# raguilar011095/planet_heightmap_generation

Measured on AMD Instinct MI355X. Metric: Mcells·iter/s, terrain-post erosion stack, higher is better.
Workload: dtype f64

## Files before the change

planet_heightmap_generation_amd/csrc/flood_host.cc:

```cpp
#include <algorithm>
#include <atomic>
#include <chrono>
#include <cmath>
#include <cstdint>
#include <cstdio>
#include <cstdlib>
#include <cstring>
#include <string>
#include <thread>
#include <stdexcept>
#include <vector>

#include "host_util.h"
#include "wo_internal.h"

namespace wo {

namespace {

inline double cell_noise(int32_t r) { return flood_cell_noise_of(r); }

using HeapItem = FloodHeapItem;
struct KeyHeap {
    hvec<HeapItem>& d;
// ... 270 lines not shown
}
void build_land_index(int32_t N, const uint8_t* ocean, FloodScratch& S) {
    S.landIndex.resize(N);
    parallel_ranges(N, [&](int64_t b, int64_t e, int) { for (int64_t r = b; r < e; ++r) S.landIndex[r] = -1; });
    parallel_ranges(S.L, [&](int64_t b, int64_t e, int) { for (int64_t i = b; i < e; ++i) S.landIndex[S.landCell[i]] = (int32_t)i; });
    filter_ranges(N, S.landByR, [&](int64_t r) { return !ocean[r]; }, [&](int64_t r) { return S.landIndex[r]; });
}
void build_compact_csr(const int32_t* off, const int32_t* adj, const uint8_t* ocean, FloodScratch& S) {
    const int32_t L = S.L;
    S.offL.assign(L + 1, 0);
    parallel_ranges(L, [&](int64_t b, int64_t e, int) {
        for (int64_t i = b; i < e; ++i) {
            const int32_t r = S.landCell[i];
            int32_t c = 0;
            for (int32_t j = off[r]; j < off[r + 1]; ++j) if (!ocean[adj[j]]) ++c;
            S.offL[i + 1] = c;
        }
    });
    inclusive_scan_parallel(S.offL.data() + 1, L);
    S.adjL.resize(S.offL[L]);
    parallel_ranges(L, [&](int64_t b, int64_t e, int) {
        for (int64_t i = b; i < e; ++i) {
            const int32_t r = S.landCell[i];
            int32_t o = S.offL[i];
            for (int32_t j = off[r]; j < off[r + 1]; ++j) { const int32_t nb = adj[j]; if (!ocean[nb]) S.adjL[o++] = S.landIndex[nb]; }
        }
    });
}
void find_seeds(int32_t N, const int32_t* off, const int32_t* adj, const uint8_t* ocean, const int32_t* label, int32_t mainLab, FloodScratch& S) {
    S.seedCell.clear();
    std::vector<std::vector<int32_t>> part(host_threads() + 1);
    parallel_ranges(N, [&](int64_t b, int64_t e, int t) {
        for (int64_t r = b; r < e; ++r) {
            if (ocean[r]) continue;
            for (int32_t j = off[r]; j < off[r + 1]; ++j) {
                const int32_t nb = adj[j];
                if (ocean[nb] && label[nb] == mainLab) { part[t].push_back(S.landIndex[r]); break; }
            }
        }
    });
    for (auto& v : part) S.seedCell.insert(S.seedCell.end(), v.begin(), v.end());
}
void build_landmass_cells(const int32_t* comp, const int32_t* compIndex, FloodScratch& S) {
    const int32_t nComp = (int32_t)S.compSize.size();
    S.compCellStart.assign(nComp + 1, 0);
    for (int32_t k = 0; k < nComp; ++k) S.compCellStart[k + 1] = S.compCellStart[k] + S.compSize[k];
    S.compCells.resize(S.compCellStart[nComp]);
    const int nt = host_threads() + 2;
    std::vector<int32_t> cnt((size_t)nt * (size_t)std::max(nComp, 1), 0);
    int usedRanges = 0;
    parallel_ranges(S.L, [&](int64_t b, int64_t e, int t) {
        int32_t* c = cnt.data() + (size_t)t * (size_t)nComp;
        for (int64_t q = b; q < e; ++q) { const int32_t k = compIndex[comp[S.landByR[q]]]; if (k >= 0) ++c[k]; }
        int cur = usedRanges; while (cur < t + 1 && !__atomic_compare_exchange_n(&usedRanges, &cur, t + 1, false, __ATOMIC_RELAXED, __ATOMIC_RELAXED)) {}
    });
    for (int32_t k = 0; k < nComp; ++k) {
        int32_t at = S.compCellStart[k];
        for (int t = 0; t < usedRanges; ++t) { int32_t& c = cnt[(size_t)t * (size_t)nComp + k]; const int32_t n = c; c = at; at += n; }
    }
    parallel_ranges(S.L, [&](int64_t b, int64_t e, int t) {
        int32_t* c = cnt.data() + (size_t)t * (size_t)nComp;
        for (int64_t q = b; q < e; ++q) { const int32_t i = S.landByR[q]; const int32_t k = compIndex[comp[i]]; if (k >= 0) S.compCells[c[k]++] = i; }
    });
}
void build_landmasses(FloodScratch& S) {
    const int32_t L = S.L;
    hvec<int32_t> comp((size_t)L);
    mesh_components(L, S.offL.data(), S.adjL.data(), [](int32_t) { return true; }, [](int32_t, int32_t) { return true; }, comp.data());
    hvec<int32_t> size((size_t)L);
    parallel_ranges(L, [&](int64_t b, int64_t e, int) { std::memset(size.data() + b, 0, sizeof(int32_t) * (size_t)(e - b)); });
    parallel_ranges(L, [&](int64_t b, int64_t e, int) { for_runs(b, e, comp.data(), [](int64_t) { return true; }, [&](int32_t root, int64_t cnt) { __atomic_fetch_add(&size[root], (int32_t)cnt, __ATOMIC_RELAXED); }); });
    const int32_t nS = (int32_t)S.seedCell.size();
    std::vector<int32_t> ord(nS);
    for (int32_t k = 0; k < nS; ++k) ord[k] = k;
    std::stable_sort(ord.begin(), ord.end(), [&](int32_t a, int32_t b) {
        const int32_t ca = comp[S.seedCell[a]], cb = comp[S.seedCell[b]];
        return size[ca] != size[cb] ? size[ca] > size[cb] : ca < cb;
    });
    S.compSeeds.assign(ord.begin(), ord.end());
    S.compSeedStart.clear(); S.compSize.clear();
    for (int32_t k = 0; k < nS; ++k)
        if (k == 0 || comp[S.seedCell[ord[k]]] != comp[S.seedCell[ord[k - 1]]]) { S.compSeedStart.push_back(k); S.compSize.push_back(size[comp[S.seedCell[ord[k]]]]); }
    S.compSeedStart.push_back(nS);
    S.stamp.resize(L);
    const int32_t nComp = (int32_t)S.compSize.size();
    hvec<int32_t>& compIndex = size;
    parallel_ranges(L, [&](int64_t b, int64_t e, int) { for (int64_t i = b; i < e; ++i) compIndex[i] = -1; });
    S.seedLocal.assign(nS, 0);
    for (int32_t k = 0; k < nComp; ++k) {
        compIndex[comp[S.seedCell[ord[S.compSeedStart[k]]]]] = k;
        for (int32_t q = S.compSeedStart[k]; q < S.compSeedStart[k + 1]; ++q) S.seedLocal[ord[q]] = q - S.compSeedStart[k];
    }
    build_landmass_cells(comp.data(), compIndex.data(), S);
}
}

void flood_build_static(int32_t N, const int32_t* off, const int32_t* adj, const float* xyz, const uint8_t* ocean, FloodScratch& S, const int32_t* mortonAll) {
    FloodTimer T(std::getenv("WO_FLOOD_TIMING") != nullptr, "[flood static]", 12);
    hvec<int32_t> label((size_t)N);
    const int32_t mainLab = main_ocean_label(N, off, adj, ocean, label.data());
    T.lap("ocean labels");
    build_land_list(N, xyz, ocean, mortonAll, S.landCell);
    T.lap("morton sort");
    const int32_t L = S.L = (int32_t)S.landCell.size();
    build_land_index(N, ocean, S);
    build_compact_csr(off, adj, ocean, S);
    T.lap("compact csr");
// ... 245 lines not shown
    j.aboveGroup = j.kx > ct.level;
    j.sameSurface = std::memcmp(&j.altSurface, &x.surface, 4) == 0;
    j.ordered = x.drain >= 0 && st[x.drain].surface < x.surface && st[ct.other].surface < x.surface;
    return j;
}
bool flood_pass1_landmasses(FloodScratch& S, FloodTieReport& rep) {
    FloodTimer T(S);
    const int32_t nComp = (int32_t)S.compSize.size();
    const int nt = flood_workers(nComp);
    rep = FloodTieReport{};
    rep.landmasses = nComp; rep.workers = nt;
    if (nComp == 0) return true;
    parallel_ranges(S.L, [&](int64_t b, int64_t en, int) { std::memset(S.stamp.data() + b, 0, sizeof(int32_t) * (size_t)(en - b)); });
    if ((int)S.workerHeaps.size() < nt) S.workerHeaps.resize(nt);
    std::vector<std::vector<Contest>> contests(nt);
    std::vector<int64_t> ng(nt, 0), nn(nt, 0);
    std::atomic<int32_t> next{0};
    auto worker = [&](int w) {
        for (;;) {
            const int32_t k = next.fetch_add(1);
            if (k >= nComp) break;
            walk_landmass(S, seeded_walk(S, k, S.workerHeaps[w], contests[w], ng[w], nn[w]));
        }
    };
    run_on_threads(nt, worker);
    for (int w = 0; w < nt; ++w) {
        rep.groups += ng[w]; rep.nested += nn[w];
        for (const Contest& ct : contests[w]) {
            ++rep.contested;
            if (ct.other >= 0 && judge_contest(S, ct).open()) { ++rep.openParents; rep.alt.push_back({ct.cell, ct.other}); }
            else ++rep.unresolved;
        }
    }
    T.lap("pass1 par");
    if (T.on) std::fprintf(stderr, "[flood] landmasses %d, workers %d, tie groups %lld (nested %lld), contested %lld, open parents %lld, unresolved %lld\n",
                           rep.landmasses, rep.workers, (long long)rep.groups, (long long)rep.nested, (long long)rep.contested, (long long)rep.openParents, (long long)rep.unresolved);
    return rep.unresolved == 0;
}
}

void flood_import_pass1(const int32_t* par, const float* surface, const int32_t* root, FloodScratch& S) {
    FloodCell* st = S.state.data();
    parallel_ranges(S.L, [&](int64_t b, int64_t en, int) {
        for (int64_t i = b; i < en; ++i) {
            const int32_t p = par[i];
            st[i].drain = (p == -2) ? TO_OCEAN : (p == -1 ? UNVISITED : p);
            st[i].surface = surface[i];
            st[i].root = (p == -1) ? -1 : root[i];
        }
    });
}

namespace {
struct TreeCtx { const FloodCell* st; float* eL; const float* surface; double carveStrength; uint8_t* onPath; int32_t* localIdx = nullptr; int32_t chainsMin = 0; };

struct ChainScratch {
    std::vector<int32_t> par, kids, kidStart, order, sz, heavy, posOf, headPos, jump, cellAt, depth;
    std::vector<float> E, S;
    std::vector<double> term;
};
bool tree_pass2_chains(const TreeCtx& X, const int32_t* cells, int32_t n, int64_t& lenSum, int64_t& nDeficit) {
    const double EPS = 1e-7;
    static thread_local ChainScratch C;
    const FloodCell* st = X.st;
    float* eL = X.eL;
    int32_t* loc = X.localIdx;
    const double carveStrength = X.carveStrength;
    auto surf = [&](int32_t i) { return X.surface ? X.surface[i] : st[i].surface; };
    for (int32_t q = 0; q < n; ++q) loc[cells[q]] = q;
    C.par.resize(n); C.kidStart.assign((size_t)n + 1, 0);
    int32_t rootQ = -1, nRoots = 0;
    for (int32_t q = 0; q < n; ++q) {
        const int32_t d = st[cells[q]].drain;
        if (d >= 0) { const int32_t pq = loc[d]; if (pq < 0 || pq >= n || cells[pq] != d) return false; C.par[q] = pq; ++C.kidStart[pq + 1]; }
        else { C.par[q] = -1; rootQ = q; ++nRoots; }
    }
    if (nRoots != 1) return false;
    if (surf(cells[rootQ]) < 0) return false;
    for (int32_t q = 0; q < n; ++q) C.kidStart[q + 1] += C.kidStart[q];
    C.kids.resize(n); C.order.resize(n);
    {
        std::vector<int32_t>& fill = C.sz; fill.assign(C.kidStart.begin(), C.kidStart.end() - 1);
        for (int32_t q = 0; q < n; ++q) if (C.par[q] >= 0) C.kids[fill[C.par[q]]++] = q;
        int32_t head = 0, tail = 0;
        C.order[tail++] = rootQ;
        while (head < tail) { const int32_t v = C.order[head++]; for (int32_t j = C.kidStart[v]; j < C.kidStart[v + 1]; ++j) C.order[tail++] = C.kids[j]; }
        if (tail != n) return false;
    }
    C.sz.assign(n, 1); C.heavy.assign(n, -1);
    for (int32_t i = n - 1; i > 0; --i) { const int32_t v = C.order[i]; C.sz[C.par[v]] += C.sz[v]; }
    for (int32_t i = 1; i < n; ++i) { const int32_t v = C.order[i], p = C.par[v]; if (C.heavy[p] < 0 || C.sz[v] > C.sz[C.heavy[p]]) C.heavy[p] = v; }
    C.posOf.resize(n); C.headPos.resize(n); C.jump.assign(n, -1); C.cellAt.resize(n); C.E.resize(n); C.S.resize(n); C.depth.resize(n);
    C.depth[rootQ] = 0;
    for (int32_t i = 1; i < n; ++i) { const int32_t v = C.order[i]; C.depth[v] = C.depth[C.par[v]] + 1; }
    {
        int32_t base = 0;
        for (int32_t i = 0; i < n; ++i) {
            const int32_t v = C.order[i];
            if (C.par[v] >= 0 && C.heavy[C.par[v]] == v) continue;
            int32_t m = 0;
            for (int32_t u = v; u >= 0; u = C.heavy[u]) ++m;
            const int32_t top = base + m - 1;
            int32_t at = top;
            for (int32_t u = v; u >= 0; u = C.heavy[u], --at) { C.posOf[u] = at; C.headPos[at] = top; C.cellAt[at] = cells[u]; C.E[at] = eL[cells[u]]; C.S[at] = surf(cells[u]); }
            C.jump[top] = C.par[v] >= 0 ? C.posOf[C.par[v]] : -1;
            base += m;
        }
// ... 23 lines not shown
                    if (!whole && S[p] <= peakElev) { scanning = false; break; }
                    if (E[p] > peakElev) { peakElev = E[p]; peakIdx = seen + (p - a); }
                }
                if (!scanning) {
                    const double rcs = std::ceil((double)len * 0.3);
                    const int32_t rad = rcs > 3.0 ? (int32_t)rcs : 3;
                    need = peakIdx + rad + 1 < len ? peakIdx + rad + 1 : len;
                }
            }
            seen += b - a + 1;
            a = jump[b];
        }
        if (X.onPath) for (int s = 0; s < nseg; ++s) for (int32_t p = segA[s]; p <= segB[s]; ++p) X.onPath[C.cellAt[p]] = 1;
        lenSum += len;
        if (peakIdx < 0) continue;
        const double carveAmount = deficit * carveStrength;
        const double rc = std::ceil((double)len * 0.3);
        const int32_t radius = rc > 3.0 ? (int32_t)rc : 3;
        const int32_t k0 = peakIdx - radius > 0 ? peakIdx - radius : 0;
        const int32_t k1 = peakIdx + radius < len - 1 ? peakIdx + radius : len - 1;
        const int32_t m = k1 - k0 + 1;
        if ((int32_t)C.term.size() < m) C.term.resize((size_t)m + 256);
        double* term = C.term.data();
        for (int32_t i = 0; i < m; ++i) term[i] = 1 - std::fabs((double)(k0 + i - peakIdx)) / (radius + 1);
        double kernelSum = 0;
        for (int32_t i = 0; i < m; ++i) kernelSum += term[i];
        if (kernelSum > 0) {
            for (int s = 0; s < nseg; ++s) {
                const int32_t ks = segK[s], ke = ks + (segB[s] - segA[s]);
                const int32_t lo = k0 > ks ? k0 : ks, hi = k1 < ke ? k1 : ke;
                float* Es = E + (segA[s] - ks);
                const double* ts = term - k0;
                for (int32_t k = lo; k <= hi; ++k) {
                    const double w = ts[k] / kernelSum;
                    float v = (float)((double)Es[k] - carveAmount * w);
                    if (v < 0) v = 0;
                    Es[k] = v;
                }
            }
        }
        E[pr] = (float)((double)E[pr] + deficit * (1 - carveStrength));
    }
    for (int32_t q = 0; q < n; ++q) eL[cells[q]] = E[C.posOf[q]];
    return true;
}

void tree_pass23(const TreeCtx& X, int32_t* cells, int32_t n, std::vector<int32_t>& path, int64_t& lenSum, int64_t& nDeficit) {
    const double EPS = 1e-7;
    const FloodCell* st = X.st;
    float* eL = X.eL;
    const double carveStrength = X.carveStrength;
    uint8_t* onPath = X.onPath;
    auto surf = [&](int32_t i) { return X.surface ? X.surface[i] : st[i].surface; };
    const bool chained = X.localIdx && X.chainsMin > 0 && n >= X.chainsMin && tree_pass2_chains(X, cells, n, lenSum, nDeficit);

    for (int32_t q = 0; q < n && !chained; ++q) {
        const int32_t r = cells[q];
        const double deficit = (double)surf(r) - (double)eL[r];
        if (deficit <= EPS) continue;
        ++nDeficit;
        path.clear();
        int32_t peakIdx = -1;
        double peakElev = -INFINITY;
        for (int32_t cur = r; cur >= 0; cur = st[cur].drain) {
            path.push_back(cur);
            if ((double)eL[cur] > peakElev) { peakElev = eL[cur]; peakIdx = (int32_t)path.size() - 1; }
        }
        if (onPath) for (int32_t c : path) onPath[c] = 1;
        const int32_t len = (int32_t)path.size();
        lenSum += len;
        if (peakIdx < 0) continue;
        const double carveAmount = deficit * carveStrength;
        const double rc = std::ceil((double)len * 0.3);
        const int32_t radius = rc > 3.0 ? (int32_t)rc : 3;
        const int32_t k0 = peakIdx - radius > 0 ? peakIdx - radius : 0;
        const int32_t k1 = peakIdx + radius < len - 1 ? peakIdx + radius : len - 1;
        double kernelSum = 0;
        for (int32_t k = k0; k <= k1; ++k) kernelSum += 1 - std::fabs((double)(k - peakIdx)) / (radius + 1);
        if (kernelSum > 0) {
            for (int32_t k = k0; k <= k1; ++k) {
                const double w = (1 - std::fabs((double)(k - peakIdx)) / (radius + 1)) / kernelSum;
                float v = (float)((double)eL[path[k]] - carveAmount * w);
                if (v < 0) v = 0;
                eL[path[k]] = v;
            }
        }
        eL[r] = (float)((double)eL[r] + deficit * (1 - carveStrength));
    }
    if (n > 1) {
        if (n <= 2048) {
            std::stable_sort(cells, cells + n, [&](int32_t a, int32_t b) { return asc_bits(surf(a)) < asc_bits(surf(b)); });
        } else {
            std::vector<uint32_t> k0(n), k1(n); std::vector<int32_t> c1(n);
            for (int32_t i = 0; i < n; ++i) k0[i] = asc_bits(surf(cells[i]));
            uint32_t* ka = k0.data(); uint32_t* kb = k1.data(); int32_t* ca = cells; int32_t* cb = c1.data();
            for (int pass = 0; pass < 3; ++pass) {
                const int sh = pass * 11; const uint32_t mask = pass == 2 ? 1023u : 2047u;
                uint32_t cnt[2049]; std::memset(cnt, 0, sizeof(cnt));
                for (int32_t i = 0; i < n; ++i) cnt[((ka[i] >> sh) & mask) + 1]++;
                for (int i = 0; i < 2048; ++i) cnt[i + 1] += cnt[i];
                for (int32_t i = 0; i < n; ++i) { const uint32_t d = cnt[(ka[i] >> sh) & mask]++; kb[d] = ka[i]; cb[d] = ca[i]; }
                std::swap(ka, kb); std::swap(ca, cb);
            }
            if (ca != cells) std::memcpy(cells, ca, sizeof(int32_t) * (size_t)n);
        }
    }
    for (int32_t q = 0; q < n; ++q) {
        const int32_t c = cells[q], t = st[c].drain;
        if (t == NO_TARGET || t == UNVISITED) continue;
        const double te = (t == TO_OCEAN) ? 0.0 : (double)eL[t];
        if ((double)eL[c] <= te) eL[c] = (float)(te + EPS);
    }
}
void cut_chunks(const std::vector<int32_t>& cnt, int32_t nTrees, int64_t budget, std::vector<int32_t>& chunkStart) {
    chunkStart.assign(1, 0);
    for (int32_t t = 0, last = 0; t < nTrees; ++t)
        if (cnt[t + 1] - cnt[last] >= budget) { chunkStart.push_back(t + 1); last = t + 1; }
    if (chunkStart.back() != nTrees) chunkStart.push_back(nTrees);
}
bool open_parent_is_harmless(const FloodScratch& S, int32_t x, int32_t p1) {
    const FloodCell* st = S.state.data(); const float* eL = S.eL.data();
    const int32_t p0 = st[x].drain;
    const bool untouched = !S.onPath[x] && std::memcmp(&eL[x], &st[x].e, 4) == 0;
    const double h = (double)st[x].e;
    return untouched && p0 >= 0 && h > (double)eL[p0] && h > (double)eL[p1];
}
void write_back(float* e, const FloodScratch& S) {
    const int32_t* landCell = S.landCell.data(); const float* eL = S.eL.data();
    if (S.landOrder) parallel_ranges(S.L, [&](int64_t b, int64_t en, int) { std::memcpy(e + b, eL + b, sizeof(float) * (size_t)(en - b)); });
    else parallel_ranges(S.L, [&](int64_t b, int64_t en, int) { for (int64_t i = b; i < en; ++i) e[landCell[i]] = eL[i]; });
}
void group_land_by_tree(FloodScratch& S, std::vector<int32_t>& cnt2) {
    const int32_t L = S.L, nTrees = (int32_t)S.seedCell.size();
    const int32_t* root = S.root.data(); const int32_t* byR = S.landByR.data(); int32_t* list2 = S.list2.data();
    cnt2.assign(nTrees + 1, 0);
    const int T = (int)std::max<int64_t>(1, std::min<int64_t>({(int64_t)host_threads(), 16, (int64_t)L / 65536 + 1}));
    std::vector<int32_t> cw((size_t)nTrees * T, 0);
    auto share = [&](int t, int64_t& b, int64_t& e) { b = (int64_t)L * t / T; e = (int64_t)L * (t + 1) / T; };
    std::vector<std::thread> th;
    for (int t = 0; t < T; ++t) th.emplace_back([&, t]() {
        int64_t b, e; share(t, b, e);
        for (int64_t k = b; k < e; ++k) { const int32_t r = root[byR[k]]; if (r >= 0) ++cw[(size_t)r * T + t]; }
    });
    for (auto& x : th) x.join();
    int32_t run = 0;
    for (int32_t tr = 0; tr < nTrees; ++tr) {
        cnt2[tr] = run;
        for (int t = 0; t < T; ++t) { const int32_t c = cw[(size_t)tr * T + t]; cw[(size_t)tr * T + t] = run; run += c; }
    }
    cnt2[nTrees] = run; th.clear();
    for (int t = 0; t < T; ++t) th.emplace_back([&, t]() {
        int64_t b, e; share(t, b, e);
        for (int64_t k = b; k < e; ++k) { const int32_t i = byR[k]; const int32_t r = root[i]; if (r >= 0) list2[cw[(size_t)r * T + t]++] = i; }
    });
    for (auto& x : th) x.join();
}
template <class Body>
// ... 124 lines not shown
        if (S.heapStore.data()[0].key > stopLevel && prefixLeft == 0) { stopped = true; break; }
        const int32_t popped = heap.pop();
        const int32_t c = popped & CELL;
        ++pops;
        {
            const FloodHeapItem* hp = S.heapStore.data();
            const size_t lim2 = heap.n < 7 ? heap.n : 7;
            for (size_t q = 0; q < lim2; ++q) {
                const int32_t raw = hp[q].cell, cc = raw & CELL;
                if (raw < 0) { __builtin_prefetch(&offL[cc]); __builtin_prefetch(&st[cc]); }
                else __builtin_prefetch(&cs[cc]);
            }
            if (heap.n > 0) {
                const int32_t raw = hp[0].cell, c0 = raw & CELL;
                if (raw < 0) for (int32_t j = offL[c0]; j < offL[c0 + 1]; ++j) __builtin_prefetch(&st[adjL[j]]);
                else __builtin_prefetch(&ci[cs[c0]]);
            }
            for (size_t q = 1; q < lim2 && q < 3; ++q) if (hp[q].cell < 0) __builtin_prefetch(&adjL[offL[hp[q].cell & CELL]]);
        }
        if (popped >= 0) {
            for (int32_t j = cs[c]; j < cs[c + 1]; ++j) heap.push(ci[j].cell, ci[j].key);
            if (prefixLeft) prefixLeft -= dirty[c] >> 1;
            continue;
        }
        ++realPops;
        const double lim = (double)st[c].surface + EPS;
        const int32_t rootC = st[c].root;
        for (int32_t i = offL[c]; i < offL[c + 1]; ++i) {
            const int32_t nb = adjL[i];
            FloodCell& sn = st[nb];
            if (sn.drain != UNVISITED) continue;
            sn.drain = c;
            sn.root = rootC;
            float k;
            if ((double)sn.e < lim) { sn.surface = (float)lim; k = (float)((double)sn.surface + cell_noise(landCell[nb])); }
            else k = (float)((double)sn.e + cell_noise(landCell[nb]));
            heap.push(nb | REAL, k);
        }
    }
    if (stopped && frontier) {
        const FloodHeapItem* hp = S.heapStore.data();
        for (size_t q = 0; q < heap.n; ++q) {
            const int32_t cc = hp[q].cell & CELL;
            if (dirty[cc]) (*frontier)[S.localIdx[cc]].push_back(FloodHeapItem{hp[q].key, cc});
        }
    }
    T.lap("replay");
    if (T.on) std::fprintf(stderr, "[flood] replay: %lld cells walked for real of %d; %s after %lld pops (level %.9g), %zu entries left in the heap\n", (long long)realPops, L,
                           stopped ? "stopped" : "ran to the end", (long long)pops, (double)stopLevel, heap.n);
    return stopped;
}

constexpr int32_t BIG = 32768, CHUNK = 4096;
struct BigJob {
    int32_t k = -1; std::vector<int32_t> cnt, chunkStart, chunkOrder; bool track = false;
    std::atomic<int> ready{0}; std::atomic<size_t> nextChunk{0}, doneChunks{0};
};
struct Round {
    const std::vector<int32_t>& list; const bool walked; const int32_t nBig;
    std::vector<BigJob> big; std::atomic<int32_t> next{0}, bigLeft;
    bool pinning = false; std::atomic<int> reservedGroup{-1};
    Round(const std::vector<int32_t>& l, bool w, int32_t nb) : list(l), walked(w), nBig(nb), big(nb), bigLeft(nb) {}
};
struct WorkerFindings { std::vector<Contest> contests; std::vector<std::pair<int32_t, int32_t>> alt; std::vector<int32_t> altComp; int64_t groups = 0, nested = 0, contested = 0, unresolved = 0; float maxLevel = -INFINITY; bool noLevel = false; };
struct PipelineCall {
    FloodScratch& S; const double carveStrength; FloodTieReport& rep; FloodTimer T; int nt;
    std::vector<WorkerFindings> loc;
    std::vector<uint8_t> dirty;
    std::vector<std::vector<int32_t>> prefix;
    Clock::time_point tRound0;
    static double ms_since(Clock::time_point t0) { return ms_between(t0, Clock::now()); }
    PipelineCall(double cs, FloodScratch& S_, FloodTieReport& rep_) : S(S_), carveStrength(cs), rep(rep_), T(S_) {
        const int32_t nComp = (int32_t)S.compSize.size();
        nt = std::min(flood_workers(std::max(nComp, 1)), std::max(1, S.L / 16384));
        rep = FloodTieReport{};
        rep.landmasses = nComp; rep.workers = nt;
        if ((int)S.workerHeaps.size() < nt) S.workerHeaps.resize(nt);
        loc.resize(nt); dirty.assign(std::max(nComp, 1), 0); prefix.resize(S.hooks.replayPrefix ? std::max(nComp, 1) : 0);
        tRound0 = Clock::now();
    }
    TreeCtx tree_ctx(bool track) const { return TreeCtx{S.state.data(), S.eL.data(), nullptr, carveStrength, track ? S.onPath.data() : nullptr, S.localIdx.data(), S.hooks.chainsMin}; }
    void place_worker(Round& R, int32_t q, AffinityScope& affinity, bool& placed) {
        const CpuGroups& cpus = CpuGroups::get();
        if (q == 0) {
            const int cpu = sched_getcpu();
            const int g = cpu >= 0 && cpu < (int)cpus.groupOf.size() ? cpus.groupOf[cpu] : -1;
            R.reservedGroup.store(g >= 0 && affinity.only(cpu) ? g : -2, std::memory_order_release);
            if (T.on) std::fprintf(stderr, "[flood] the largest walk stays on cpu %d; the other workers keep off its L3 (group %d of %zu)\n", cpu, g, cpus.groups.size());
            placed = true;
        } else {
            const int g = R.reservedGroup.load(std::memory_order_acquire);
            if (g >= 0) { (void)affinity.all_but_group(cpus, g); placed = true; }
            else if (g == -2) placed = true;
        }
    }
    bool walk_and_judge(int w, int32_t q, int32_t k, bool& track) {
        WorkerFindings& me = loc[w];
        static thread_local PopLog popLog;
        PopLog* const log = prefix.empty() ? nullptr : &popLog;
        const int32_t forceDirty = S.hooks.forceDirty;
        const bool largest = T.on && q == 0;
        me.contests.clear();
        const auto tw0 = Clock::now();
        WalkStats ws;
        Walk walk = seeded_walk(S, k, S.workerHeaps[w], me.contests, me.groups, me.nested);
        walk.log = log; walk.stats = largest ? &ws : nullptr;
        walk_landmass(S, walk);
        if (log && (!me.contests.empty() || q == forceDirty)) {
            const int32_t len = q == forceDirty && me.contests.empty() ? (int32_t)((int64_t)log->n * S.hooks.forcePrefixPermille / 1000) : log->prefix;
            prefix[k].assign(log->cells.begin(), log->cells.begin() + len);
            if (T.on) std::fprintf(stderr, "[flood] landmass %d (%d cells): %d pops before its first tie group with a contested cell\n", k, S.compSize[k], len);
        }
        if (largest) std::fprintf(stderr, "[flood] walk of the largest landmass (%d cells): %.1f ms; heap mean %lld max %lld entries, %lld pops below the level reached, %lld raised keys, %d seeds\n", S.compSize[k], ms_since(tw0),
                                  (long long)(ws.heapSum / std::max<int64_t>(ws.pops, 1)), (long long)ws.heapMax, (long long)ws.descending, (long long)ws.raised, walk.nSeeds);
        const size_t alt0 = me.alt.size();
        bool undecided = false;
        for (const Contest& ct : me.contests) {
            ++me.contested;
            bool open = false;
            if (ct.other < 0) me.noLevel = true;
            else {
                if (ct.level > me.maxLevel) me.maxLevel = ct.level;
                const ContestJudgement j = judge_contest(S, ct);
                open = j.open();
                if (!open && T.on) std::fprintf(stderr, "[flood] undecided contested cell %d (other %d): %s%s%s level %.9g key %.9g surface %.9g / %.9g e %.9g\n", S.landCell[ct.cell], S.landCell[ct.other],
                                                j.aboveGroup ? "" : "cascades-inside-the-group ", j.sameSurface ? "" : "surface-differs ", j.ordered ? "" : "pass3-order ", (double)ct.level, (double)j.kx,
                                                (double)S.state[ct.cell].surface, (double)j.altSurface, (double)S.state[ct.cell].e);
            }
            if (open) { me.alt.push_back({ct.cell, ct.other}); me.altComp.push_back(k); track = true; }
            else { ++me.unresolved; undecided = true; }
        }
        if (q == forceDirty) undecided = true;
        if (undecided) { me.alt.resize(alt0); me.altComp.resize(alt0); dirty[k] = 1; }
        return undecided;
    }
    void group_by_tree(int32_t k, std::vector<int32_t>& c) {
        const FloodCell* st = S.state.data(); int32_t* list2 = S.list2.data();
        const int32_t base = S.compCellStart[k], n = S.compCellStart[k + 1] - base, nTrees = S.compSeedStart[k + 1] - S.compSeedStart[k];
        const int32_t* cells = S.compCells.data() + base;
        c.assign((size_t)nTrees + 1, 0);
        for (int32_t qq = 0; qq < n; ++qq) ++c[S.seedLocal[st[cells[qq]].root] + 1];
        for (int32_t t = 0; t < nTrees; ++t) c[t + 1] += c[t];
        static thread_local std::vector<int32_t> pos;
        pos.assign(c.begin(), c.end() - 1);
        for (int32_t qq = 0; qq < n; ++qq) { const int32_t i = cells[qq]; list2[base + pos[S.seedLocal[st[i].root]]++] = i; }
    }
    void publish_big_job(BigJob& J, int32_t k, bool track) {
        const std::vector<int32_t>& c = J.cnt; J.k = k; J.track = track;
        cut_chunks(c, S.compSeedStart[k + 1] - S.compSeedStart[k], CHUNK, J.chunkStart);
        J.chunkOrder.resize(J.chunkStart.size() - 1);
        for (size_t x = 0; x < J.chunkOrder.size(); ++x) J.chunkOrder[x] = (int32_t)x;
        std::stable_sort(J.chunkOrder.begin(), J.chunkOrder.end(), [&](int32_t x, int32_t y) { return c[J.chunkStart[x + 1]] - c[J.chunkStart[x]] > c[J.chunkStart[y + 1]] - c[J.chunkStart[y]]; });
        J.ready.store(1, std::memory_order_release);
    }
    void run_chunks(Round& R, BigJob& J, std::vector<int32_t>& path) {
        const TreeCtx ctx = tree_ctx(J.track);
        const size_t nChunks = J.chunkStart.size() - 1;
        int32_t* trees = S.list2.data() + S.compCellStart[J.k];
        for (;;) {
            const size_t cq = J.nextChunk.fetch_add(1);
            if (cq >= nChunks) break;
            const size_t c = (size_t)J.chunkOrder[cq];
            int64_t a = 0, b = 0;
            for (int32_t t = J.chunkStart[c]; t < J.chunkStart[c + 1]; ++t)
                if (J.cnt[t + 1] > J.cnt[t]) {
                    const int32_t nT = J.cnt[t + 1] - J.cnt[t];
                    const bool timed = T.on && nT >= 16384;
                    const auto tt0 = timed ? Clock::now() : tRound0;
                    const int64_t a0 = a, b0 = b;
                    tree_pass23(ctx, trees + J.cnt[t], nT, path, a, b);
                    if (timed) std::fprintf(stderr, "[flood] landmass %d: tree of %d cells, passes 2+3 %.2f ms (%lld deficit cells, %lld path steps), done at %.1f ms\n", J.k, nT,
                                            ms_since(tt0), (long long)(b - b0), (long long)(a - a0), ms_since(tRound0));
                }
            if (J.doneChunks.fetch_add(1) + 1 == nChunks) R.bigLeft.fetch_sub(1);
        }
    }
    void help_until_done(Round& R, std::vector<int32_t>& path) {
        while (R.bigLeft.load() > 0) {
            bool did = false;
            for (BigJob& J : R.big)
                if (J.ready.load(std::memory_order_acquire) && J.nextChunk.load() < J.chunkStart.size() - 1) { run_chunks(R, J, path); did = true; }
            if (!did) std::this_thread::sleep_for(std::chrono::microseconds(25));
        }
    }
    void worker(Round& R, int w) {
        std::vector<int32_t> path, cnt;
        AffinityScope affinity; bool placed = false;
        for (;;) {
            const int32_t q = R.next.fetch_add(1);
            if (q >= (int32_t)R.list.size()) break;
            const int32_t k = R.list[q];
            if (R.pinning && !placed) place_worker(R, q, affinity, placed);
            bool track = false;
            const bool undecided = !R.walked && walk_and_judge(w, q, k, track);
            const bool isBig = q < R.nBig;
            if (undecided) {
                if (isBig) { BigJob& J = R.big[q]; J.k = k; J.chunkStart.assign(1, 0); J.ready.store(1, std::memory_order_release); R.bigLeft.fetch_sub(1); }
                continue;
            }
            std::vector<int32_t>& c = isBig ? R.big[q].cnt : cnt;
            group_by_tree(k, c);
            if (T.on && q == 0) std::fprintf(stderr, "[flood] largest landmass: walk + contests + tree lists done at %.1f ms\n", ms_since(tRound0));
            if (isBig) { publish_big_job(R.big[q], k, track); run_chunks(R, R.big[q], path); }
            else {
                const TreeCtx ctx = tree_ctx(track);
                int32_t* trees = S.list2.data() + S.compCellStart[k]; int64_t a = 0, b = 0;
                for (size_t t = 0; t + 1 < c.size(); ++t) if (c[t + 1] > c[t]) tree_pass23(ctx, trees + c[t], c[t + 1] - c[t], path, a, b);
            }
        }
        help_until_done(R, path);
    }
    void run_round(const std::vector<int32_t>& list, bool walked) {
        const int32_t nList = (int32_t)list.size(); int32_t nBig = 0;
        while (nBig < nList && S.compSize[list[nBig]] >= BIG) ++nBig;
        Round R(list, walked, nBig);
        R.pinning = S.hooks.pin && !walked && nBig > 0 && nt > 1 && !CpuGroups::get().groups.empty();
        const int use = std::min(nt, std::max(1, nList));
        if (T.on) std::fprintf(stderr, "[flood] round setup done at %.1f ms\n", ms_since(tRound0));
        if (use == 1 && nBig == 0) worker(R, 0);
        else {
            const int th_n = nBig > 0 ? nt : use;
            parallel_ranges((int64_t)th_n, [&](int64_t b, int64_t en, int) { for (int64_t w = b; w < en; ++w) worker(R, (int)w); }, 1);
        }
        if (T.on) std::fprintf(stderr, "[flood] round joined at %.1f ms\n", ms_since(tRound0));
    }
    void recheck_open_parents(int64_t& pathRedo) {
        for (const WorkerFindings& l : loc)
            for (size_t a = 0; a < l.alt.size(); ++a)
                if (!open_parent_is_harmless(S, l.alt[a].first, l.alt[a].second) && !dirty[l.altComp[a]]) { dirty[l.altComp[a]] = 1; ++pathRedo; }
        for (const WorkerFindings& l : loc) { rep.groups += l.groups; rep.nested += l.nested; rep.contested += l.contested; rep.unresolved += l.unresolved; rep.openParents += (int64_t)l.alt.size(); }
    }
    std::vector<int32_t> landmasses_to_replay() {
        if (std::find(dirty.begin(), dirty.end(), 1) != dirty.end()) for (const WorkerFindings& l : loc) for (int32_t k : l.altComp) dirty[k] = 1;
        std::vector<int32_t> redo;
        for (int32_t k = 0; k < (int32_t)S.compSize.size(); ++k) if (dirty[k]) redo.push_back(k);
        return redo;
    }
    float replay_stop_level() const {
        float stopLevel = -INFINITY;
        bool toTheEnd = S.hooks.forceDirty >= 0;
        for (const WorkerFindings& l : loc) { if (l.noLevel) toTheEnd = true; if (l.maxLevel > stopLevel) stopLevel = l.maxLevel; }
        if (toTheEnd) stopLevel = INFINITY;
        return S.hooks.hasReplayStop ? S.hooks.replayStop : stopLevel;
    }
    void replay(const std::vector<int32_t>& redo) {
        const float stopLevel = replay_stop_level();
        const std::vector<std::vector<int32_t>>* pre = prefix.empty() ? nullptr : &prefix;
        std::vector<std::vector<FloodHeapItem>> frontier(S.compSize.size());
        if (!replay_dirty_landmasses(S, dirty, stopLevel, &frontier, pre)) return;
        std::atomic<int> contestedAgain{0};
        const FloodCell* st = S.state.data(); uint8_t* seen = S.seen.data(); int32_t* stamp = S.stamp.data();
        parallel_ranges((int64_t)redo.size(), [&](int64_t b, int64_t en, int) {
            for (int64_t q = b; q < en; ++q) {
                const int32_t k = redo[q];
                const int32_t* cells = S.compCells.data() + S.compCellStart[k];
                const int32_t n = S.compCellStart[k + 1] - S.compCellStart[k];
                for (int32_t x = 0; x < n; ++x) { const int32_t i = cells[x]; seen[i] = st[i].drain != UNVISITED; stamp[i] = 0; }
                static thread_local hvec<FloodHeapItem> store;
// ... 17 lines not shown
    const std::vector<int32_t> redo = P.landmasses_to_replay();
    rep.replayed = (int32_t)redo.size();
    if (!redo.empty() && !replayAllowed) return false;
    if (P.T.on) std::fprintf(stderr, "[flood] landmasses %d, workers %d, tie groups %lld (nested %lld), contested %lld, open parents %lld, undecided %lld -> %d landmasses through the replay\n",
                             rep.landmasses, rep.workers, (long long)rep.groups, (long long)rep.nested, (long long)rep.contested, (long long)rep.openParents, (long long)rep.unresolved, rep.replayed);
    if (!redo.empty()) {
        P.replay(redo);
        P.run_round(redo, true);
        P.T.lap("round 2");
    }
    write_back(e, S);
    P.T.lap("writeback");
    return true;
}

void count_ties(FloodHostStats& st, const FloodTieReport& rep) { st.tieGroups += rep.groups; st.contested += rep.contested; st.openParents += rep.openParents; st.unresolved += rep.unresolved; }
bool timed_pipeline(float* e, double carveStrength, FloodScratch& S, FloodHostStats& st, FloodTieReport& rep, bool replayAllowed) {
    const auto t0 = Clock::now();
    const bool done = flood_landmass_pipeline(e, carveStrength, S, rep, st.pathRedo, replayAllowed);
    st.pass1Ms += ms_between(t0, Clock::now());
    if (replayAllowed && rep.replayed) { ++st.replays; st.replayedLandmasses += rep.replayed; }
    return done;
}
void exchange_own_positions(int32_t N, const FloodScratch& S, FloodExchange& X) {
    X.ownPos.resize((size_t)S.L);
    const uint8_t* toc = X.trueOcean.data(); const int32_t* li = S.landIndex.data();
    int32_t cnt = 0, lowest = -1, placed = 0;
    for (int32_t r = 0; r < N; ++r) if (!toc[r]) { if (li[r] >= 0) { X.ownPos[(size_t)li[r]] = cnt; ++placed; if (lowest < 0) lowest = r; } ++cnt; }
    if (placed != S.L) throw std::runtime_error("flood exchange: the resident ocean mask has land cells that the planet's true mask (wo_planet_set_flood_exchange) calls ocean");
    X.landTotal = cnt; X.minOwnCell = lowest; X.posVersion = S.staticVersion;
}

void exchange_flood_planet(int32_t N, const int32_t* off, const int32_t* adj, const float* xyz, float* snap, float* pack, double carveStrength, FloodHostStats& st, FloodExchange& X) {
    ++X.globalFloods;
    FloodScratch& G = X.global;
    if (!G.staticValid || G.staticN != N) flood_build_static(N, off, adj, xyz, X.trueOcean.data(), G);
    flood_gather(snap, G);
    FloodTieReport rep;
    timed_pipeline(snap, carveStrength, G, st, rep, true);
    const int32_t* gCell = G.landCell.data(); const int32_t* byR = G.landByR.data();
    parallel_ranges(G.L, [&](int64_t b, int64_t en, int) { for (int64_t q = b; q < en; ++q) pack[q] = snap[gCell[byR[q]]]; });
}
enum class HostRoute { Pipeline, TwoPhase, Serial };
}

void flood_host_passes(float* e, double carveStrength, FloodScratch& S, FloodHostStats* stats) {
    static const HostRoute route = [] {
        const char* v = std::getenv("WO_FLOOD_HOST"); const std::string r = v ? v : "";
        return r == "serial" ? HostRoute::Serial : r == "two-phase" ? HostRoute::TwoPhase : HostRoute::Pipeline;
    }();
    FloodHostStats local;
    FloodHostStats& st = stats ? *stats : local;
    ++st.calls;
    flood_gather(e, S);
    bool done = false;
    if (route != HostRoute::Serial) {
        FloodTieReport rep;
        if (route == HostRoute::TwoPhase) {
            const auto t0 = Clock::now();
            const bool exact = flood_pass1_landmasses(S, rep);
            const auto t1 = Clock::now();
            st.pass1Ms += ms_between(t0, t1);
            if (exact) {
                done = flood_pass23_host(e, carveStrength, S, &rep.alt);
                st.pass23Ms += ms_between(t1, Clock::now());
                if (!done) ++st.pathRedo;
            }
        } else done = timed_pipeline(e, carveStrength, S, st, rep, true);
        count_ties(st, rep);
        if (!done) flood_gather(e, S);
    }
    if (!done) {
        const auto t0 = Clock::now();
        flood_pass1_host(S);
        const auto t1 = Clock::now();
        flood_pass23_host(e, carveStrength, S);
        st.pass1Ms += ms_between(t0, t1); st.pass23Ms += ms_between(t1, Clock::now());
        ++st.serialPass1;
    }
}

int flood_host_passes_exchange(int32_t N, const int32_t* off, const int32_t* adj, const float* xyz, float* e, double carveStrength,
                               FloodScratch& S, FloodHostStats* stats, FloodExchange& X) {
    FloodHostStats local;
    FloodHostStats& st = stats ? *stats : local;
    ++st.calls; ++X.calls;
    X.snapshot.resize((size_t)N);
    float* snap = X.snapshot.data();
    parallel_ranges(N, [&](int64_t b, int64_t en, int) { std::memcpy(snap + b, e + b, sizeof(float) * (size_t)(en - b)); });
    bool mine = false;
    if (S.L > 0) {
        flood_gather(e, S);
        FloodTieReport rep;
        mine = !timed_pipeline(e, carveStrength, S, st, rep, false);
        count_ties(st, rep);
    }
    if (S.L > 0 && (X.posVersion != S.staticVersion || X.ownPos.size() != (size_t)S.L)) exchange_own_positions(N, S, X);
    const int32_t bid = mine ? INT32_MAX - X.minOwnCell : 0;
    int32_t flag = bid;
    if (int rc = X.fn(X.user, 0, &flag, 1)) return rc;
    if (!flag) return 0;
    ++X.gathers;
    if (int rc = X.fn(X.user, 1, snap, N)) return rc;
    if (X.landTotal < 0) { int64_t cnt = 0; for (int32_t r = 0; r < N; ++r) cnt += X.trueOcean[r] ? 0 : 1; X.landTotal = cnt; }
    X.landPack.resize((size_t)std::max<int64_t>(X.landTotal, 1));
    float* pack = X.landPack.data();
    if (mine && flag == bid) {
// ... 22 lines not shown
```

Measured before the change: 6417.

## Share big-landmass tree grouping and pass-3 sorts across idle host workers

Grouping a big landmass's cells by tree is now split into three phases (histogram, prefix, scatter) that idle workers can join through a shared job. Large per-tree pass-3 sorts are posted to a slot board so helpers can run them while the owner does pass 2, and the sort scratch buffers become thread-local. Idle helpers now spin briefly instead of sleeping once the largest landmass has been walked. This aims to cut the serial tail on the host flood pipeline, at the cost of extra spin-waiting, atomics and an added copy of the sorted cells.

```diff
diff --git a/planet_heightmap_generation_amd/csrc/flood_host.cc b/planet_heightmap_generation_amd/csrc/flood_host.cc
--- a/planet_heightmap_generation_amd/csrc/flood_host.cc
+++ b/planet_heightmap_generation_amd/csrc/flood_host.cc
@@ -346,7 +346,7 @@
     parallel_ranges(S.L, [&](int64_t b, int64_t e, int t) {
         int32_t* c = cnt.data() + (size_t)t * (size_t)nComp;
         for (int64_t q = b; q < e; ++q) { const int32_t k = compIndex[comp[S.landByR[q]]]; if (k >= 0) ++c[k]; }
-        int cur = usedRanges; while (cur < t + 1 && !__atomic_compare_exchange_n(&usedRanges, &cur, t + 1, false, __ATOMIC_RELAXED, __ATOMIC_RELAXED)) {}
+        int cur = __atomic_load_n(&usedRanges, __ATOMIC_RELAXED); while (cur < t + 1 && !__atomic_compare_exchange_n(&usedRanges, &cur, t + 1, false, __ATOMIC_RELAXED, __ATOMIC_RELAXED)) {}
     });
     for (int32_t k = 0; k < nComp; ++k) {
         int32_t at = S.compCellStart[k];
@@ -698,7 +698,68 @@
 }
 
 namespace {
-struct TreeCtx { const FloodCell* st; float* eL; const float* surface; double carveStrength; uint8_t* onPath; int32_t* localIdx = nullptr; int32_t chainsMin = 0; };
+struct SortBoard;
+struct TreeCtx { const FloodCell* st; float* eL; const float* surface; double carveStrength; uint8_t* onPath; int32_t* localIdx = nullptr; int32_t chainsMin = 0; SortBoard* board = nullptr; };
+inline void cpu_relax() {
+#if defined(__x86_64__) || defined(__i386__)
+    __builtin_ia32_pause();
+#else
+    std::this_thread::yield();
+#endif
+}
+
+void pass3_order(const TreeCtx& X, const int32_t* in, int32_t n, int32_t* out) {
+    auto surf = [&](int32_t i) { return X.surface ? X.surface[i] : X.st[i].surface; };
+    if (n <= 2048) {
+        std::memcpy(out, in, sizeof(int32_t) * (size_t)n);
+        std::stable_sort(out, out + n, [&](int32_t a, int32_t b) { return asc_bits(surf(a)) < asc_bits(surf(b)); });
+        return;
+    }
+    static thread_local std::vector<uint32_t> k0, k1; static thread_local std::vector<int32_t> c1;
+    if ((int32_t)k0.size() < n) { k0.resize(n); k1.resize(n); c1.resize(n); }
+    for (int32_t i = 0; i < n; ++i) k0[i] = asc_bits(surf(in[i]));
+    const uint32_t* const ksrc[3] = {k0.data(), k1.data(), k0.data()}; uint32_t* const kdst[3] = {k1.data(), k0.data(), k1.data()};
+    const int32_t* const csrc[3] = {in, out, c1.data()}; int32_t* const cdst[3] = {out, c1.data(), out};
+    for (int pass = 0; pass < 3; ++pass) {
+        const int sh = pass * 11; const uint32_t mask = pass == 2 ? 1023u : 2047u;
+        const uint32_t* ka = ksrc[pass]; uint32_t* kb = kdst[pass]; const int32_t* ca = csrc[pass]; int32_t* cb = cdst[pass];
+        uint32_t cnt[2049]; std::memset(cnt, 0, sizeof(cnt));
+        for (int32_t i = 0; i < n; ++i) cnt[((ka[i] >> sh) & mask) + 1]++;
+        for (int i = 0; i < 2048; ++i) cnt[i + 1] += cnt[i];
+        for (int32_t i = 0; i < n; ++i) { const uint32_t d = cnt[(ka[i] >> sh) & mask]++; kb[d] = ka[i]; cb[d] = ca[i]; }
+    }
+}
+struct SortBoard {
+    struct Slot { std::atomic<int> state{0}; const TreeCtx* X = nullptr; const int32_t* in = nullptr; int32_t n = 0; int32_t* out = nullptr; };
+    static constexpr int SLOTS = 32;
+    Slot slot[SLOTS];
+    Slot* post(const TreeCtx& X, const int32_t* in, int32_t n, int32_t* out) {
+        for (Slot& s : slot) {
+            int free = 0;
+            if (s.state.load(std::memory_order_relaxed) != 0 || !s.state.compare_exchange_strong(free, 1, std::memory_order_acquire)) continue;
+            s.X = &X; s.in = in; s.n = n; s.out = out;
+            s.state.store(2, std::memory_order_release);
+            return &s;
+        }
+        return nullptr;
+    }
+    bool help() {
+        for (Slot& s : slot) {
+            int posted = 2;
+            if (s.state.load(std::memory_order_relaxed) != 2 || !s.state.compare_exchange_strong(posted, 3, std::memory_order_acquire)) continue;
+            pass3_order(*s.X, s.in, s.n, s.out);
+            s.state.store(4, std::memory_order_release);
+            return true;
+        }
+        return false;
+    }
+    void collect(Slot* s) {
+        int posted = 2;
+        if (s->state.compare_exchange_strong(posted, 1, std::memory_order_acquire)) pass3_order(*s->X, s->in, s->n, s->out);
+        else while (s->state.load(std::memory_order_acquire) != 4) cpu_relax();
+        s->state.store(0, std::memory_order_release);
+    }
+};
 
 struct ChainScratch {
     std::vector<int32_t> par, kids, kidStart, order, sz, heavy, posOf, headPos, jump, cellAt, depth;
@@ -828,6 +889,9 @@
     const double carveStrength = X.carveStrength;
     uint8_t* onPath = X.onPath;
     auto surf = [&](int32_t i) { return X.surface ? X.surface[i] : st[i].surface; };
+    static thread_local std::vector<int32_t> sorted;
+    if (n > 1 && (int32_t)sorted.size() < n) sorted.resize((size_t)n + 1024);
+    SortBoard::Slot* const slot = X.board && n > 1 && X.chainsMin > 0 && n >= X.chainsMin ? X.board->post(X, cells, n, sorted.data()) : nullptr;
     const bool chained = X.localIdx && X.chainsMin > 0 && n >= X.chainsMin && tree_pass2_chains(X, cells, n, lenSum, nDeficit);
 
     for (int32_t q = 0; q < n && !chained; ++q) {
@@ -864,21 +928,10 @@
         eL[r] = (float)((double)eL[r] + deficit * (1 - carveStrength));
     }
     if (n > 1) {
-        if (n <= 2048) {
-            std::stable_sort(cells, cells + n, [&](int32_t a, int32_t b) { return asc_bits(surf(a)) < asc_bits(surf(b)); });
-        } else {
-            std::vector<uint32_t> k0(n), k1(n); std::vector<int32_t> c1(n);
-            for (int32_t i = 0; i < n; ++i) k0[i] = asc_bits(surf(cells[i]));
-            uint32_t* ka = k0.data(); uint32_t* kb = k1.data(); int32_t* ca = cells; int32_t* cb = c1.data();
-            for (int pass = 0; pass < 3; ++pass) {
-                const int sh = pass * 11; const uint32_t mask = pass == 2 ? 1023u : 2047u;
-                uint32_t cnt[2049]; std::memset(cnt, 0, sizeof(cnt));
-                for (int32_t i = 0; i < n; ++i) cnt[((ka[i] >> sh) & mask) + 1]++;
-                for (int i = 0; i < 2048; ++i) cnt[i + 1] += cnt[i];
-                for (int32_t i = 0; i < n; ++i) { const uint32_t d = cnt[(ka[i] >> sh) & mask]++; kb[d] = ka[i]; cb[d] = ca[i]; }
-                std::swap(ka, kb); std::swap(ca, cb);
-            }
-            if (ca != cells) std::memcpy(cells, ca, sizeof(int32_t) * (size_t)n);
+        if (!slot && n <= 2048) std::stable_sort(cells, cells + n, [&](int32_t a, int32_t b) { return asc_bits(surf(a)) < asc_bits(surf(b)); });
+        else {
+            if (slot) X.board->collect(slot); else pass3_order(X, cells, n, sorted.data());
+            std::memcpy(cells, sorted.data(), sizeof(int32_t) * (size_t)n);
         }
     }
     for (int32_t q = 0; q < n; ++q) {
@@ -1109,15 +1162,25 @@
 }
 
 constexpr int32_t BIG = 32768, CHUNK = 4096;
+struct GroupJob {
+    int32_t base = 0, n = 0, nTrees = 0, ranges = 0;
+    std::vector<int32_t> hist;
+    std::atomic<int> phase{0};
+    std::atomic<int32_t> next[3], done[3];
+    GroupJob() { for (int p = 0; p < 3; ++p) { next[p].store(0); done[p].store(0); } }
+};
 struct BigJob {
     int32_t k = -1; std::vector<int32_t> cnt, chunkStart, chunkOrder; bool track = false;
     std::atomic<int> ready{0}; std::atomic<size_t> nextChunk{0}, doneChunks{0};
+    GroupJob group;
 };
 struct Round {
     const std::vector<int32_t>& list; const bool walked; const int32_t nBig;
     std::vector<BigJob> big; std::atomic<int32_t> next{0}, bigLeft;
     bool pinning = false; std::atomic<int> reservedGroup{-1};
-    Round(const std::vector<int32_t>& l, bool w, int32_t nb) : list(l), walked(w), nBig(nb), big(nb), bigLeft(nb) {}
+    std::atomic<bool> largestWalked;
+    SortBoard board;
+    Round(const std::vector<int32_t>& l, bool w, int32_t nb) : list(l), walked(w), nBig(nb), big(nb), bigLeft(nb), largestWalked(w) {}
 };
 struct WorkerFindings { std::vector<Contest> contests; std::vector<std::pair<int32_t, int32_t>> alt; std::vector<int32_t> altComp; int64_t groups = 0, nested = 0, contested = 0, unresolved = 0; float maxLevel = -INFINITY; bool noLevel = false; };
 struct PipelineCall {
@@ -1136,7 +1199,7 @@
         loc.resize(nt); dirty.assign(std::max(nComp, 1), 0); prefix.resize(S.hooks.replayPrefix ? std::max(nComp, 1) : 0);
         tRound0 = Clock::now();
     }
-    TreeCtx tree_ctx(bool track) const { return TreeCtx{S.state.data(), S.eL.data(), nullptr, carveStrength, track ? S.onPath.data() : nullptr, S.localIdx.data(), S.hooks.chainsMin}; }
+    TreeCtx tree_ctx(bool track, Round& R) const { return TreeCtx{S.state.data(), S.eL.data(), nullptr, carveStrength, track ? S.onPath.data() : nullptr, S.localIdx.data(), S.hooks.chainsMin, R.nBig > 0 ? &R.board : nullptr}; }
     void place_worker(Round& R, int32_t q, AffinityScope& affinity, bool& placed) {
         const CpuGroups& cpus = CpuGroups::get();
         if (q == 0) {
@@ -1202,6 +1265,56 @@
         pos.assign(c.begin(), c.end() - 1);
         for (int32_t qq = 0; qq < n; ++qq) { const int32_t i = cells[qq]; list2[base + pos[S.seedLocal[st[i].root]]++] = i; }
     }
+    void group_task(BigJob& J, int ph, int32_t task) {
+        GroupJob& G = J.group;
+        const FloodCell* st = S.state.data(); const int32_t* seedLocal = S.seedLocal.data();
+        const int32_t* cells = S.compCells.data() + G.base;
+        const int64_t R = G.ranges;
+        if (ph == 2) {
+            int32_t* c = J.cnt.data();
+            for (int32_t t = (int32_t)((int64_t)G.nTrees * task / R), te = (int32_t)((int64_t)G.nTrees * (task + 1) / R); t < te; ++t) {
+                int32_t run = 0;
+                for (int64_t p = 0; p < R; ++p) { int32_t& h = G.hist[(size_t)p * G.nTrees + t]; const int32_t v = h; h = run; run += v; }
+                c[t + 1] = run;
+            }
+            return;
+        }
+        int32_t* h = G.hist.data() + (size_t)task * G.nTrees;
+        const int32_t b = (int32_t)((int64_t)G.n * task / R), e = (int32_t)((int64_t)G.n * (task + 1) / R);
+        if (ph == 1) {
+            std::memset(h, 0, sizeof(int32_t) * (size_t)G.nTrees);
+            for (int32_t qq = b; qq < e; ++qq) ++h[seedLocal[st[cells[qq]].root]];
+        } else {
+            const int32_t* c = J.cnt.data(); int32_t* list2 = S.list2.data() + G.base;
+            for (int32_t qq = b; qq < e; ++qq) { const int32_t i = cells[qq], t = seedLocal[st[i].root]; list2[c[t] + h[t]++] = i; }
+        }
+    }
+    bool help_group(BigJob& J) {
+        GroupJob& G = J.group;
+        const int ph = G.phase.load(std::memory_order_acquire);
+        if (ph < 1 || ph > 3 || G.next[ph - 1].load(std::memory_order_relaxed) >= G.ranges) return false;
+        bool did = false;
+        for (int32_t task; (task = G.next[ph - 1].fetch_add(1, std::memory_order_relaxed)) < G.ranges; did = true) {
+            group_task(J, ph, task);
+            G.done[ph - 1].fetch_add(1, std::memory_order_release);
+        }
+        return did;
+    }
+    void group_by_tree_shared(BigJob& J, int32_t k) {
+        GroupJob& G = J.group;
+        G.base = S.compCellStart[k]; G.n = S.compCellStart[k + 1] - G.base; G.nTrees = S.compSeedStart[k + 1] - S.compSeedStart[k];
+        G.ranges = (int32_t)std::max<int64_t>(1, std::min<int64_t>({(int64_t)nt, (int64_t)G.n / 8192, 4 * (int64_t)G.n / std::max(G.nTrees, 1)}));
+        G.hist.resize((size_t)G.ranges * G.nTrees);
+        J.cnt.assign((size_t)G.nTrees + 1, 0);
+        for (int ph = 1; ph <= 3; ++ph) {
+            G.phase.store(ph, std::memory_order_release);
+            help_group(J);
+            while (G.done[ph - 1].load(std::memory_order_acquire) < G.ranges) cpu_relax();
+            if (ph == 2) for (int32_t t = 0; t < G.nTrees; ++t) J.cnt[t + 1] += J.cnt[t];
+        }
+        G.phase.store(4, std::memory_order_release);
+        if (T.on) std::fprintf(stderr, "[flood] landmass %d: %d cells grouped by tree in %d shared ranges (%d trees), done at %.1f ms\n", k, G.n, G.ranges, G.nTrees, ms_since(tRound0));
+    }
     void publish_big_job(BigJob& J, int32_t k, bool track) {
         const std::vector<int32_t>& c = J.cnt; J.k = k; J.track = track;
         cut_chunks(c, S.compSeedStart[k + 1] - S.compSeedStart[k], CHUNK, J.chunkStart);
@@ -1211,7 +1324,7 @@
         J.ready.store(1, std::memory_order_release);
     }
     void run_chunks(Round& R, BigJob& J, std::vector<int32_t>& path) {
-        const TreeCtx ctx = tree_ctx(J.track);
+        const TreeCtx ctx = tree_ctx(J.track, R);
         const size_t nChunks = J.chunkStart.size() - 1;
         int32_t* trees = S.list2.data() + S.compCellStart[J.k];
         for (;;) {
@@ -1233,11 +1346,18 @@
         }
     }
     void help_until_done(Round& R, std::vector<int32_t>& path) {
+        constexpr int SPINS = 4096;
+        int idle = 0;
         while (R.bigLeft.load() > 0) {
             bool did = false;
-            for (BigJob& J : R.big)
+            for (BigJob& J : R.big) {
+                if (help_group(J)) did = true;
                 if (J.ready.load(std::memory_order_acquire) && J.nextChunk.load() < J.chunkStart.size() - 1) { run_chunks(R, J, path); did = true; }
-            if (!did) std::this_thread::sleep_for(std::chrono::microseconds(25));
+            }
+            if (R.board.help()) did = true;
+            if (did) idle = 0;
+            else if (R.largestWalked.load(std::memory_order_acquire) && idle < SPINS) { ++idle; cpu_relax(); }
+            else std::this_thread::sleep_for(std::chrono::microseconds(25));
         }
     }
     void worker(Round& R, int w) {
@@ -1250,17 +1370,18 @@
             if (R.pinning && !placed) place_worker(R, q, affinity, placed);
             bool track = false;
             const bool undecided = !R.walked && walk_and_judge(w, q, k, track);
+            if (q == 0) R.largestWalked.store(true, std::memory_order_release);
             const bool isBig = q < R.nBig;
             if (undecided) {
                 if (isBig) { BigJob& J = R.big[q]; J.k = k; J.chunkStart.assign(1, 0); J.ready.store(1, std::memory_order_release); R.bigLeft.fetch_sub(1); }
                 continue;
             }
             std::vector<int32_t>& c = isBig ? R.big[q].cnt : cnt;
-            group_by_tree(k, c);
+            if (isBig) group_by_tree_shared(R.big[q], k); else group_by_tree(k, c);
             if (T.on && q == 0) std::fprintf(stderr, "[flood] largest landmass: walk + contests + tree lists done at %.1f ms\n", ms_since(tRound0));
             if (isBig) { publish_big_job(R.big[q], k, track); run_chunks(R, R.big[q], path); }
             else {
-                const TreeCtx ctx = tree_ctx(track);
+                const TreeCtx ctx = tree_ctx(track, R);
                 int32_t* trees = S.list2.data() + S.compCellStart[k]; int64_t a = 0, b = 0;
                 for (size_t t = 0; t + 1 < c.size(); ++t) if (c[t + 1] > c[t]) tree_pass23(ctx, trees + c[t], c[t + 1] - c[t], path, a, b);
             }
@@ -1384,7 +1505,9 @@
     FloodHostStats local;
     FloodHostStats& st = stats ? *stats : local;
     ++st.calls;
+    const auto tCall0 = Clock::now();
     flood_gather(e, S);
+    struct CallLap { const FloodScratch& S; Clock::time_point t0; ~CallLap() { if (S.hooks.timing) std::fprintf(stderr, "[flood] whole call %8.1f ms\n", ms_between(t0, Clock::now())); } } callLap{S, tCall0};
     bool done = false;
     if (route != HostRoute::Serial) {
         FloodTieReport rep;
diff --git a/profiles/flood_host_probe.py b/profiles/flood_host_probe.py
--- /dev/null
+++ b/profiles/flood_host_probe.py
@@ -0,0 +1,137 @@
+import argparse
+import ctypes as C
+import os
+import re
+import statistics
+import subprocess
+import sys
+import tempfile
+import time
+from pathlib import Path
+
+import numpy as np
+
+REPO = Path(__file__).resolve().parents[1]
+sys.path.insert(0, str(REPO))
+ERODE_ITERS = 4
+PARAMS = dict(K=3e-4, m=0.5, dt=1.0, talus=1.16, kThermal=0.015, glacialStrength=0.5)
+LAPS = (("walk", r"walk of the largest landmass \(\d+ cells\): ([0-9.]+) ms"),
+        ("tree_lists_at", r"walk \+ contests \+ tree lists done at ([0-9.]+) ms"),
+        ("joined_at", r"round joined at ([0-9.]+) ms"),
+        ("pipeline", r"\[flood\] pipeline\s+([0-9.]+) ms"),
+        ("call", r"\[flood\] whole call\s+([0-9.]+) ms"))
+RAW_LOG = None
+
+
+def P(a):
+    return a.ctypes.data_as(C.c_void_p)
+
+
+def timed_calls(emu, mesh, xyz, e0, oc, cs, calls):
+    e = e0.copy()
+    st = np.zeros(11)
+    with tempfile.TemporaryFile() as f:
+        sys.stderr.flush()
+        saved = os.dup(2)
+        os.dup2(f.fileno(), 2)
+        try:
+            emu.emu_flood_host(mesh.numRegions, P(mesh.adjOffset), P(mesh.adjList), P(xyz), P(e), P(oc), cs, 11, calls, P(st))
+        finally:
+            os.dup2(saved, 2)
+            os.close(saved)
+        f.seek(0)
+        log = f.read().decode(errors="replace")
+    if RAW_LOG:
+        with open(RAW_LOG, "a") as f:
+            f.write(f"==== carve {cs}\n{log}")
+    rows = {name: [float(x) for x in re.findall(rx, log)] for name, rx in LAPS}
+    largest = re.search(r"walk of the largest landmass \((\d+) cells\)", log)
+    return e, rows, int(largest.group(1)) if largest else 0, st
+
+
+def report(title, rows, calls, out):
+    n = min((len(v) for v in rows.values() if v), default=0)
+    lines = [title]
+    if n == 0:
+        lines.append("  no laps in the log (WO_FLOOD_TIMING lines missing)")
+    else:
+        cols = [k for k, v in rows.items() if len(v) >= n]
+        table = {k: rows[k][-n:] for k in cols}
+        if "pipeline" in table and "walk" in table:
+            table["tail"] = [p - w for p, w in zip(table["pipeline"], table["walk"])]
+        lines.append("  call  " + "  ".join(f"{k:>13}" for k in table))
+        for i in range(n):
+            lines.append(f"  {i:4d}  " + "  ".join(f"{table[k][i]:13.1f}" for k in table))
+        lines.append("  med   " + "  ".join(f"{statistics.median(table[k]):13.1f}" for k in table))
+        lines.append("  min   " + "  ".join(f"{min(table[k]):13.1f}" for k in table))
+        lines.append("  max   " + "  ".join(f"{max(table[k]):13.1f}" for k in table))
+    text = "\n".join(lines)
+    print(text, flush=True)
+    if out:
+        with open(out, "a") as f:
+            f.write(text + "\n")
+
+
+def main():
+    ap = argparse.ArgumentParser()
+    ap.add_argument("--cells", type=int, default=10_000_000)
+    ap.add_argument("--seed", type=int, default=1)
+    ap.add_argument("--calls", type=int, default=7)
+    ap.add_argument("--cache", default=tempfile.gettempdir())
+    ap.add_argument("--label", default="")
+    ap.add_argument("--out", default=None)
+    ap.add_argument("--keep-landmasses", type=int, default=0, help="K > 0: every landmass but the K largest becomes ocean (for hosts with few cores)")
+    ap.add_argument("--no-build", action="store_true", help="use the emulator and oracle libraries as they are")
+    ap.add_argument("--lib", default=None, help="another build of tests/emu's libemu.so (A/B against the tree's)")
+    ap.add_argument("--log", default=None, help="append the library's whole timing log to this file")
+    args = ap.parse_args()
+    global RAW_LOG
+    RAW_LOG = args.log
+    os.environ["WO_FLOOD_TIMING"] = "1"
+    if not args.no_build:
+        subprocess.run(["make", "-s", "-C", str(REPO / "tests" / "emu")], check=True)
+        subprocess.run(["make", "-s", "-C", str(REPO / "oracle")], check=True)
+    from oracle import pyoracle as O
+    from planet_heightmap_generation_amd import sphere_mesh as S
+    emu = C.CDLL(args.lib or str(REPO / "tests" / "emu" / "_build" / "libemu.so"))
+    p = C.c_void_p
+    emu.emu_flood_host.argtypes = [C.c_int32, p, p, p, p, p, C.c_double, C.c_int32, C.c_int32, p]
+    t0 = time.time()
+    mesh, xyz, nd = S.build_sphere(args.cells, 0.75, args.seed)
+    om = O.Mesh(mesh.adjOffset, mesh.adjList)
+    first = Path(args.cache) / f"flood_host_probe_first_{mesh.numRegions}_{args.seed}.npy"
+    if first.exists():
+        e0 = np.load(first)
+    else:
+        e0 = O.warp_terrain(om, O.synthetic_terrain(xyz, args.seed), xyz, args.seed, 0.75)
+        np.save(first, e0)
+    oc = (e0 <= 0).astype(np.uint8)
+    if args.keep_landmasses > 0:
+        from planet_heightmap_generation_amd import decomposed as D
+        label = D.land_components(mesh, oc)
+        labs, counts = np.unique(label[label >= 0], return_counts=True)
+        kept = labs[np.argsort(-counts, kind="stable")[:args.keep_landmasses]]
+        oc = np.where(np.isin(label, kept), 0, 1).astype(np.uint8)
+    head = (f"== {args.label or 'flood_host_probe'}: {mesh.numRegions} cells, seed {args.seed}, {int((oc == 0).sum())} land cells, {args.calls} calls per field, "
+            f"host threads {os.environ.get('WO_HOST_THREADS', 'default')}, flood threads {os.environ.get('WO_FLOOD_THREADS', 'default')}, {os.cpu_count()} CPUs "
+            f"(inputs in {time.time() - t0:.0f} s); ms")
+    print(head, flush=True)
+    if args.out:
+        with open(args.out, "a") as f:
+            f.write(head + "\n")
+    e1, rows, largest, _ = timed_calls(emu, mesh, xyz, e0, oc, 0.5, args.calls)
+    report(f"first flood (carve 0.5), largest landmass {largest} cells", rows, args.calls, args.out)
+    cache = Path(args.cache) / f"flood_host_probe_second_{mesh.numRegions}_{args.seed}_{ERODE_ITERS}_{args.keep_landmasses}.npy"
+    if cache.exists():
+        e2 = np.load(cache)
+    else:
+        t0 = time.time()
+        e2 = O.erode_composite(om, e1, xyz, oc, ERODE_ITERS, PARAMS["K"], PARAMS["m"], PARAMS["dt"], ERODE_ITERS, PARAMS["talus"], PARAMS["kThermal"], 0, PARAMS["glacialStrength"], nd)
+        np.save(cache, e2)
+        print(f"second-flood-like field: {ERODE_ITERS} oracle iterations in {time.time() - t0:.0f} s, cached in {cache}", flush=True)
+    _, rows, largest, _ = timed_calls(emu, mesh, xyz, e2, oc, 0.85, args.calls)
+    report(f"second-flood-like field ({ERODE_ITERS} oracle iterations after the first flood; carve 0.85), largest landmass {largest} cells", rows, args.calls, args.out)
+
+
+if __name__ == "__main__":
+    main()
```

Result: no change. 6447 (median of 2 runs) (+0.5%).
